# SUNGBEOMCHOI/Rubiks-Cube-Solver

Hardware: NVIDIA B200
Metric: cube transitions/sec (higher is better)
Workload: dtype u8

## Files before the change

rubiks_cube_solver_b200/csrc/cube_sched.cuh:

```cuda
#pragma once
#include <cstdint>
#include <cuda_runtime.h>

namespace sched {

constexpr int kClaimChunk = 2;
constexpr int kRanges = 8;
constexpr int kTailDiv = 4;
constexpr int kSlots = 1024;
constexpr int kExhausted = 0x7fffff00;

struct Slot { unsigned next[kRanges][32]; unsigned ctas_done; unsigned tail_div; unsigned pad[30]; };

Slot* claim_slot();
int tail_div();

struct WarpTiles {
    Slot* slot;
    int n_tiles, total_warps, tail0;
    int next_static;
    int r, visited;
    int cur, end;
    int chunk;
    unsigned pending;

    __device__ __forceinline__ int lo(int range) const
    {
        return tail0 + (int)((long long)range * (n_tiles - tail0) / kRanges);
    }
    __device__ __forceinline__ void claim_ahead(int lane)
    {
        if (lane == 0) pending = atomicAdd(&slot->next[r][0], (unsigned)chunk);
    }

    __device__ __forceinline__ void init(Slot* s, int n, int warps_per_cta, int warp, int lane, int tail_div,
                                         int claim_chunk = kClaimChunk)
    {
        slot = s; n_tiles = n; total_warps = (int)gridDim.x * warps_per_cta; chunk = claim_chunk;
        const int gid = (int)blockIdx.x * warps_per_cta + warp;
        tail0 = tail_div > 0 ? n - n / tail_div : n;
        next_static = gid;
        r = gid % kRanges; visited = 0; cur = end = 0; pending = 0;
        if (next_static >= tail0) claim_ahead(lane);
    }

    __device__ __forceinline__ int pop(int lane)
    {
        if (next_static < tail0) {
            const int t = next_static;
            next_static += total_warps;
            if (next_static >= tail0) claim_ahead(lane);
            return t;
        }
        while (cur >= end) {
            if (visited >= kRanges) return kExhausted;
            const unsigned got = __shfl_sync(0xffffffffu, pending, 0);
            const int hi = lo(r + 1);
            const long long base = (long long)lo(r) + got;
            if (base < hi) {
                cur = (int)base;
                end = cur + chunk < hi ? cur + chunk : hi;
            } else {
                bool left = false;
                if (lane < kRanges) left = lo(lane) + (long long)__ldcg(&slot->next[lane][0]) < lo(lane + 1);
                const unsigned open = __ballot_sync(0xffffffffu, left) & ((1u << kRanges) - 1u);
                if (open == 0) { visited = kRanges; return kExhausted; }
                const unsigned rot = (open >> (r + 1)) | (open << (kRanges - r - 1));
                r = (r + 1 + (__ffs(rot & ((1u << kRanges) - 1u)) - 1)) % kRanges;
            }
            claim_ahead(lane);
        }
        return cur++;
    }
};

__device__ __forceinline__ void release(Slot* slot)
{
    if (threadIdx.x == 0) {
        __threadfence();
        if (atomicAdd(&slot->ctas_done, 1u) == gridDim.x - 1) {
            for (int i = 0; i < kRanges; ++i) slot->next[i][0] = 0;
            slot->ctas_done = 0;
            __threadfence();
        }
    }
}

}
```

rubiks_cube_solver_b200/csrc/cube_threads.cuh:

```cuda
#pragma once
#include <cstdlib>
#include "cube_common.cuh"

template <int SIZE>
CUBE_HD void scramble_apply_word(CubieState& st, const uint32_t* s_tbl, uint32_t w)
{
    const uint32_t w4 = (w * 4u) & 0x3c3c3c3cu;
#pragma unroll
    for (int k = 0; k < 4; ++k) cubie_move_at<SIZE>(st, s_tbl, cube_prmt(w4, 0u, 0x4440u + k));
}

template <int SIZE>
CUBE_HD void scramble_run_staged(CubieState& st, int tid, int depth, const uint8_t* s_moves, const uint32_t* s_tbl)
{
    const uint32_t* mw = reinterpret_cast<const uint32_t*>(s_moves);
    const uint32_t r = (uint32_t)tid * (uint32_t)depth;
    const uint32_t wi = r >> 2, sh = (r & 3u) << 3;
    const int nfull = depth >> 2, tail = depth & 3;
    uint32_t lo = mw[wi];
#pragma unroll 2
    for (int j = 0; j < nfull; ++j) {
        const uint32_t hi = mw[wi + j + 1];
        const uint32_t w = cube_funnel_r(lo, hi, sh);
        lo = hi;
// ... 190 lines not shown
        const uint32_t m0 = cube_prmt(s.e0, t0, cube_hi16(Q.x)) ^ (P.w & 0x10101010u);
        const uint32_t m1 = cube_prmt(s.e1, t1, cube_hi16(Q.y)) ^ Q.w;
        const uint32_t m2 = cube_prmt(s.e2, t2, cube_hi16(Q.z)) ^ (P.w & 0x20202020u);
        s.e0 = m0; s.e1 = m1; s.e2 = m2;
    } else {
        uint32_t sel, t0w;
        tbl.ld64(addr, sel, t0w);
        const uint32_t t1w = tbl.ld32(addr + roff);
        const uint32_t n0 = cube_prmt(s.c0, s.c1, sel) + t0w;
        const uint32_t n1 = cube_prmt(s.c0, s.c1, cube_hi16(sel)) + t1w;
        s.c0 = n0; s.c1 = n1;
    }
}

template <int SIZE, int DEPTH>
CUBE_HD constexpr int pair_static_shift(int k)
{
    return DEPTH <= 0 ? -1
         : SIZE == 3 ? ((2 * DEPTH) % 4 == 0 ? ((k * DEPTH) % 4) * 8 : -1)
                     : (DEPTH % 4 == 0 ? 0 : -1);
}

template <int SSH>
CUBE_HD uint32_t pair_rows_word(uint32_t lo, uint32_t hi, uint32_t sh)
{
    constexpr uint32_t K = (uint32_t)(CUBE_PAIR_BASE + 256);
    if (SSH == 0) return lo * K;
    if (SSH == 16) return hi * (K << 16) + cube_hi16(lo) * K;
    return cube_funnel_r(lo, hi, sh) * K;
}

template <int SIZE, int DEPTH, int NS, class TBL>
CUBE_HD void scramble_pairs_run(CubieState (&st)[NS], const int (&rows)[NS], int depth_rt, const uint8_t* s_moves,
                                const TBL& tbl, uint32_t lanereg, uint32_t roff)
{
    const int depth = DEPTH > 0 ? DEPTH : depth_rt;
    const uint32_t* mw = reinterpret_cast<const uint32_t*>(s_moves);
    const int nfull = depth >> 2, tail = depth & 3;
    uint32_t wi[NS], sh[NS], lo[NS];
#pragma unroll
    for (int k = 0; k < NS; ++k) {
        const uint32_t r = (uint32_t)rows[k] * (uint32_t)depth;
        wi[k] = r >> 2; sh[k] = (r & 3u) << 3;
        lo[k] = mw[wi[k]];
    }
    auto word = [&](int j) {
        uint32_t y[NS];
        static_assert(NS == 1 || NS % 2 == 0, "instances come in pairs");
        if (SIZE == 3 || NS <= 2) {
            {
                constexpr int s0 = (NS >= 2) ? pair_static_shift<SIZE, DEPTH>(0) : -1;
#pragma unroll
                for (int h = 0; h < NS; h += 2) {
                    const uint32_t hi = (s0 == 0) ? 0u : mw[wi[h] + j + 1];
                    y[h] = pair_rows_word<s0>(lo[h], hi, sh[h]);
                    lo[h] = (s0 == 0) ? mw[wi[h] + j + 1] : hi;
                }
            }
            if (NS >= 2) {
                constexpr int s1 = pair_static_shift<SIZE, DEPTH>(1);
#pragma unroll
                for (int h = 1; h < NS; h += 2) {
                    const uint32_t hi = (s1 == 0) ? 0u : mw[wi[h] + j + 1];
                    y[h] = pair_rows_word<s1>(lo[h], hi, sh[h]);
                    lo[h] = (s1 == 0) ? mw[wi[h] + j + 1] : hi;
                }
            }
        } else {
            constexpr int s = pair_static_shift<2, DEPTH>(0);
#pragma unroll
            for (int k = 0; k < NS; ++k) {
                const uint32_t hi = (s == 0) ? 0u : mw[wi[k] + j + 1];
                y[k] = pair_rows_word<s>(lo[k], hi, sh[k]);
                lo[k] = (s == 0) ? mw[wi[k] + j + 1] : hi;
            }
        }
#pragma unroll
        for (int k = 0; k < NS; ++k) pair_apply<SIZE>(st[k], tbl, pair_addr<0>(y[k], lanereg), roff);
#pragma unroll
        for (int k = 0; k < NS; ++k) pair_apply<SIZE>(st[k], tbl, pair_addr<1>(y[k], lanereg), roff);
    };
    auto fold = [&]() {
#pragma unroll
        for (int k = 0; k < NS; ++k) {
            st[k].c0 = cubie_fold_twist(st[k].c0);
            st[k].c1 = cubie_fold_twist(st[k].c1);
        }
    };
    if (DEPTH > 0) {
#pragma unroll
        for (int j = 0; j < DEPTH / 4; ++j) {
            word(j);
            if (DEPTH > 30 && (j % 5 == 4 || j == DEPTH / 4 - 1)) fold();
        }
    } else {
        int j = 0;
        for (; j + 5 <= nfull; j += 5) {
            word(j); word(j + 1); word(j + 2); word(j + 3); word(j + 4);
            fold();
        }
        for (; j < nfull; ++j) word(j);
    }
    if (tail) {
        const uint32_t keep = (1u << (8 * tail)) - 1u;
        uint32_t y[NS];
#pragma unroll
        for (int k = 0; k < NS; ++k) {
            const uint32_t w = (cube_funnel_r(lo[k], mw[wi[k] + nfull + 1], sh[k]) & keep) | (0x0c0c0c0cu & ~keep);
            y[k] = w * (uint32_t)(CUBE_PAIR_BASE + 256);
        }
#pragma unroll
        for (int k = 0; k < NS; ++k) pair_apply<SIZE>(st[k], tbl, pair_addr<0>(y[k], lanereg), roff);
        if (tail == 3) {
#pragma unroll
            for (int k = 0; k < NS; ++k) pair_apply<SIZE>(st[k], tbl, pair_addr<1>(y[k], lanereg), roff);
        }
    }
}

template <int SIZE, int NS, class TBL>
CUBE_HD void scramble_pairs_run_units(CubieState (&st)[NS], const uint32_t (&base)[NS], const uint32_t (&shift)[NS], int len,
                                      const uint8_t* s_moves, const TBL& tbl, uint32_t lanereg, uint32_t roff)
{
    constexpr uint32_t K = (uint32_t)(CUBE_PAIR_BASE + 256);
    auto fold = [&]() {
#pragma unroll
        for (int k = 0; k < NS; ++k) {
            st[k].c0 = cubie_fold_twist(st[k].c0);
            st[k].c1 = cubie_fold_twist(st[k].c1);
        }
    };
    auto word = [&](const uint32_t (&w)[NS], bool second) {
        uint32_t y[NS];
#pragma unroll
        for (int k = 0; k < NS; ++k) y[k] = w[k] * K;
#pragma unroll
        for (int k = 0; k < NS; ++k) pair_apply<SIZE>(st[k], tbl, pair_addr<0>(y[k], lanereg), roff);
        if (second) {
#pragma unroll
            for (int k = 0; k < NS; ++k) pair_apply<SIZE>(st[k], tbl, pair_addr<1>(y[k], lanereg), roff);
        }
    };
    auto aligned = [&](const CubeVec4& a, const CubeVec4& b, uint32_t sh, uint32_t (&o)[4]) {
        const bool q0 = (sh & 4u) != 0, q1 = (sh & 8u) != 0;
        const uint32_t c[8] = {a.x, a.y, a.z, a.w, b.x, b.y, b.z, b.w};
        uint32_t e[7], d[5];
#pragma unroll
        for (int j = 0; j < 7; ++j) e[j] = q0 ? c[j + 1] : c[j];
#pragma unroll
        for (int j = 0; j < 5; ++j) d[j] = q1 ? e[j + 2] : e[j];
        const uint32_t r = (sh & 3u) << 3;
#pragma unroll
        for (int j = 0; j < 4; ++j) o[j] = cube_funnel_r(d[j], d[j + 1], r);
    };
    fold();
    CubeVec4 cur[NS];
#pragma unroll
    for (int k = 0; k < NS; ++k) cur[k] = cube_ld128(s_moves + base[k]);
    int g = 0;
    for (; g + 16 <= len; g += 16) {
        CubeVec4 nxt[NS];
        uint32_t m[NS][4], w[NS];
#pragma unroll
        for (int k = 0; k < NS; ++k) {
            nxt[k] = cube_ld128(s_moves + base[k] + g + 16);
            aligned(cur[k], nxt[k], shift[k], m[k]);
            cur[k] = nxt[k];
        }
#pragma unroll
        for (int j = 0; j < 4; ++j) {
#pragma unroll
            for (int k = 0; k < NS; ++k) w[k] = m[k][j];
            word(w, true);
        }
        fold();
    }
    const int rem = len - g;
    if (rem) {
        uint32_t m[NS][4], w[NS];
#pragma unroll
        for (int k = 0; k < NS; ++k) {
            const CubeVec4 nxt = cube_ld128(s_moves + base[k] + g + 16);
            aligned(cur[k], nxt, shift[k], m[k]);
        }
        const int nwords = rem >> 2, tail = rem & 3;
#pragma unroll
        for (int j = 0; j < 3; ++j) {
            if (j < nwords) {
#pragma unroll
                for (int k = 0; k < NS; ++k) w[k] = m[k][j];
                word(w, true);
            }
        }
        if (tail) {
            const uint32_t keep = (1u << (8 * tail)) - 1u;
#pragma unroll
            for (int k = 0; k < NS; ++k) {
                const uint32_t t = nwords == 0 ? m[k][0] : nwords == 1 ? m[k][1] : nwords == 2 ? m[k][2] : m[k][3];
                w[k] = (t & keep) | (0x0c0c0c0cu & ~keep);
            }
            word(w, tail == 3);
        }
    }
}

template <int SIZE, class TBL>
CUBE_HD void scramble_pairs_last(CubieState& st, uint32_t action, const TBL& tbl, uint32_t lanereg, uint32_t roff)
{
    st.c0 = cubie_fold_twist(st.c0);
    st.c1 = cubie_fold_twist(st.c1);
    const uint32_t y = (action | 0x0c0c0c00u) * (uint32_t)(CUBE_PAIR_BASE + 256);
    pair_apply<SIZE>(st, tbl, pair_addr<0>(y, lanereg), roff);
}

CUBE_HD uint32_t cube_swz128(uint32_t f) { return f ^ ((f >> 3) & 0x70u); }

template <int SIZE, int NS, class TBL>
CUBE_HD void scramble_pairs_run_swizzled(CubieState (&st)[NS], const uint8_t* tile, int lane, int depth, const TBL& tbl,
                                         uint32_t lanereg, uint32_t roff)
{
    constexpr uint32_t K = (uint32_t)(CUBE_PAIR_BASE + 256);
    static_assert(SIZE == 2 || NS == 2, "3x3x3: two rows per lane");
    auto word = [&](const uint32_t (&w)[NS]) {
        uint32_t y[NS];
#pragma unroll
        for (int k = 0; k < NS; ++k) y[k] = w[k] * K;
#pragma unroll
        for (int k = 0; k < NS; ++k) pair_apply<SIZE>(st[k], tbl, pair_addr<0>(y[k], lanereg), roff);
#pragma unroll
        for (int k = 0; k < NS; ++k) pair_apply<SIZE>(st[k], tbl, pair_addr<1>(y[k], lanereg), roff);
    };
    auto fold = [&]() {
#pragma unroll
        for (int k = 0; k < NS; ++k) {
            st[k].c0 = cubie_fold_twist(st[k].c0);
            st[k].c1 = cubie_fold_twist(st[k].c1);
        }
    };
    auto unit = [&](uint32_t f) { return cube_ld128(tile + cube_swz128(f)); };
    if (SIZE == 3 && (depth & 8)) {
        const int a = depth >> 4;
        const uint32_t f0 = (uint32_t)(lane * 2 * depth);
        CubeVec4 p = unit(f0 + 16 * a);
        const uint32_t last0[2] = {p.x, p.y};
        auto word2 = [&](uint32_t w0, uint32_t w1) {
            uint32_t w[NS];
            w[0] = w0; w[NS - 1] = w1;
            word(w);
        };
        for (int g = 0; g < a; ++g) {
            const CubeVec4 v = unit(f0 + 16 * g), q = unit(f0 + 16 * (a + g + 1));
            word2(v.x, p.z);
            word2(v.y, p.w);
            word2(v.z, q.x);
            word2(v.w, q.y);
            p = q;
            fold();
        }
        word2(last0[0], p.z);
        word2(last0[1], p.w);
        return;
    }
    uint32_t f[NS];
#pragma unroll
    for (int k = 0; k < NS; ++k) f[k] = (uint32_t)((SIZE == 3 ? 2 * lane + k : lane + 32 * k) * depth);
    for (int g = 0; g < depth; g += 16) {
        CubeVec4 v[NS];
#pragma unroll
        for (int k = 0; k < NS; ++k) v[k] = unit(f[k] + g);
        uint32_t w[NS];
#pragma unroll
        for (int k = 0; k < NS; ++k) w[k] = v[k].x;
        word(w);
#pragma unroll
        for (int k = 0; k < NS; ++k) w[k] = v[k].y;
        word(w);
#pragma unroll
        for (int k = 0; k < NS; ++k) w[k] = v[k].z;
        word(w);
#pragma unroll
        for (int k = 0; k < NS; ++k) w[k] = v[k].w;
        word(w);
        fold();
    }
}

CUBE_HD uint32_t cube_shr1(uint32_t x)
{
#if defined(__CUDA_ARCH__)
    uint32_t r;
    asm("mul.hi.u32 %0, %1, 2147483648;" : "=r"(r) : "r"(x));
    return r;
#else
    return x >> 1;
#endif
}

CUBE_HD uint32_t cubie_canonical_flip(uint32_t e)
{
    return ((cube_shr1(e) & 0x10101010u) ^ e) & 0x1f1f1f1fu;
}

template <int SIZE, class LUT>
CUBE_HD bool scramble_pairs_finish(CubieState& st, int row, const LUT& lut, uint8_t* s_out)
{
    st.c0 = cubie_reduce_twist(st.c0);
    st.c1 = cubie_reduce_twist(st.c1);
    bool ok = (st.c0 == 0x03020100u) & (st.c1 == 0x07060504u);
    uint32_t L[20];
#pragma unroll
    for (int q = 0; q < 4; ++q) {
        L[q] = lut.corner(st.c0, q);
        L[4 + q] = lut.corner(st.c1, q);
    }
    if (SIZE == 3) {
        const uint32_t f0 = cubie_canonical_flip(st.e0), f1 = cubie_canonical_flip(st.e1), f2 = cubie_canonical_flip(st.e2);
        ok = ok && ((f0 == 0x03020100u) & (f1 == 0x07060504u) & (f2 == 0x0b0a0908u));
        L[8] = lut.template edge<0>(f0);   L[9] = lut.template edge<1>(f0);   L[10] = lut.template edge<2>(f0);  L[11] = lut.template edge<3>(f0);
        L[12] = lut.template edge<4>(f1);  L[13] = lut.template edge<5>(f1);  L[14] = lut.template edge<6>(f1);  L[15] = lut.template edge<7>(f1);
        L[16] = lut.template edge<8>(f2);  L[17] = lut.template edge<9>(f2);  L[18] = lut.template edge<10>(f2); L[19] = lut.template edge<11>(f2);
        uint32_t w[13], h;
        uint8_t* rowp = s_out + 54 * row;
        if (row & 1) {
            cube_assemble3_odd(L, w, &h);
            *reinterpret_cast<uint16_t*>(rowp) = (uint16_t)h;
            uint32_t* wb = reinterpret_cast<uint32_t*>(rowp + 2);
#pragma unroll
            for (int j = 0; j < 13; ++j) wb[j] = w[j];
        } else {
            cube_assemble3_even(L, w, &h);
            uint32_t* wb = reinterpret_cast<uint32_t*>(rowp);
#pragma unroll
            for (int j = 0; j < 13; ++j) wb[j] = w[j];
            *reinterpret_cast<uint16_t*>(rowp + 52) = (uint16_t)h;
        }
    } else {
        uint32_t w[6];
        cube_assemble2(L, w);
        uint64_t* rowp = reinterpret_cast<uint64_t*>(s_out + 24 * row);
#pragma unroll
        for (int j = 0; j < 3; ++j) rowp[j] = (uint64_t)w[2 * j] | ((uint64_t)w[2 * j + 1] << 32);
    }
    return ok;
}

template <int SIZE>
CUBE_HD uint32_t pair_row_bit(uint32_t m0, uint32_t m1, int row)
{
    if (SIZE == 3) return (((row & 1) ? m1 : m0) >> (row >> 1)) & 1u;
    return (((row & 32) ? m1 : m0) >> (row & 31)) & 1u;
}

template <int SIZE>
CUBE_HD uint32_t pair_solved_word(uint32_t m0, uint32_t m1, int k)
{
    return pair_row_bit<SIZE>(m0, m1, 4 * k) | pair_row_bit<SIZE>(m0, m1, 4 * k + 1) << 8 |
           pair_row_bit<SIZE>(m0, m1, 4 * k + 2) << 16 | pair_row_bit<SIZE>(m0, m1, 4 * k + 3) << 24;
}

template <int SIZE>
CUBE_HD void walk_turn(uint8_t* row, uint32_t m, const uint32_t* s_cyc)
{
#pragma unroll
    for (int c = 0; c < CubeGeom<SIZE>::NCYC; ++c) {
        const uint32_t w = s_cyc[c * CUBE_MOVE_ROWS + m];
        const uint32_t a = w & 0xffu, b = (w >> 8) & 0xffu, cc = (w >> 16) & 0xffu, d = w >> 24;
        const uint8_t vb = row[b], vc = row[cc], vd = row[d], va = row[a];
        row[a] = vb; row[b] = vc; row[cc] = vd; row[d] = va;
    }
}

template <int SIZE>
CUBE_HD bool row_solved(const uint8_t* row)
{
    constexpr int S = CubeGeom<SIZE>::S, K = S / 6;
    const uint16_t* h = reinterpret_cast<const uint16_t*>(row);
    uint32_t diff = 0;
    uint32_t prev = 0;
#pragma unroll
    for (int i = 0; i < S / 2; ++i) {
        const uint32_t cur = h[i];
        const uint32_t b0 = cur & 0xffu, b1 = cur >> 8;
        if ((2 * i) % K != 0) diff |= b0 ^ prev;
        if ((2 * i + 1) % K != 0) diff |= b1 ^ b0;
        prev = b1;
    }
    return diff == 0;
}


template <int SIZE> struct WalkImage { static constexpr int W = (SIZE == 3) ? 14 : 6; };

CUBE_HD uint32_t walk_private_off(int k) { return (uint32_t)((k >> 2) * 128 + (k & 3)); }

CUBE_HD void walk_cycle_entry(uint32_t cw, int shift, uint32_t* e)
{
    const int a = (int)(cw & 0xffu) + shift, b = (int)((cw >> 8) & 0xffu) + shift;
    const int c = (int)((cw >> 16) & 0xffu) + shift, d = (int)(cw >> 24) + shift;
    e[0] = walk_private_off(a) | walk_private_off(b) << 16;
    e[1] = walk_private_off(c) | walk_private_off(d) << 16;
}

template <int SIZE>
CUBE_HD void walk_turn_private(uint8_t* lane_base, const uint32_t* ent, uint32_t m)
{
#pragma unroll
    for (int c = 0; c < CubeGeom<SIZE>::NCYC; ++c) {
        const uint32_t w0 = ent[(c * CUBE_MOVE_ROWS + m) * 2], w1 = ent[(c * CUBE_MOVE_ROWS + m) * 2 + 1];
        const uint32_t a = w0 & 0xffffu, b = cube_hi16(w0), cc = w1 & 0xffffu, d = cube_hi16(w1);
        const uint8_t vb = lane_base[b], vc = lane_base[cc], vd = lane_base[d], va = lane_base[a];
        lane_base[a] = vb; lane_base[b] = vc; lane_base[cc] = vd; lane_base[d] = va;
    }
}

template <int A>
CUBE_HD void walk_select_child2(const uint32_t* p, uint32_t m, uint32_t* out)
{
    uint32_t c[6];
    cube_child2<A>(p, c);
#pragma unroll
    for (int j = 0; j < 6; ++j) out[j] = (m == (uint32_t)A) ? c[j] : out[j];
}

CUBE_HD void walk_turn_registers2(uint32_t* w, uint32_t m)
{
    uint32_t out[6];
#pragma unroll
    for (int j = 0; j < 6; ++j) out[j] = w[j];
    walk_select_child2<0>(w, m, out);
    walk_select_child2<1>(w, m, out);
    walk_select_child2<2>(w, m, out);
    walk_select_child2<3>(w, m, out);
    walk_select_child2<4>(w, m, out);
    walk_select_child2<5>(w, m, out);
#pragma unroll
    for (int j = 0; j < 6; ++j) w[j] = out[j];
}

template <int SIZE, int SHIFT>
CUBE_HD bool image_solved(const uint32_t* w)
{
    constexpr int S = CubeGeom<SIZE>::S, K = S / 6, W = WalkImage<SIZE>::W;
    uint32_t acc = 0;
#pragma unroll
    for (int j = 0; j < W; ++j) {
        uint32_t mask = 0;
#pragma unroll
        for (int k = 0; k < 4; ++k) {
            const int i = 4 * j + k - SHIFT;
            if (i >= 1 && i < S && (i % K) != 0) mask |= 0xffu << (8 * k);
        }
        if (mask) {
            const uint32_t prev = (j == 0) ? (w[0] << 8) : ((w[j] << 8) | (w[j - 1] >> 24));
            acc |= (w[j] ^ prev) & mask;
        }
    }
    return acc == 0;
}

template <int DTYPE> struct OneHot;
template <> struct OneHot<0> { static constexpr int V = 8, ESIZE = 2; };
template <> struct OneHot<1> { static constexpr int V = 4, ESIZE = 4; };
template <> struct OneHot<2> { static constexpr int V = 16, ESIZE = 1; };

template <int DTYPE>
CUBE_HD void onehot_set(uint32_t* w, int p)
{
    if (DTYPE == 0) {
        const uint32_t v = (p & 1) ? 0x3f800000u : 0x00003f80u;
#pragma unroll
        for (int q = 0; q < 4; ++q) w[q] |= ((p >> 1) == q) ? v : 0u;
    } else if (DTYPE == 1) {
#pragma unroll
        for (int q = 0; q < 4; ++q) w[q] |= (p == q) ? 0x3f800000u : 0u;
    } else {
        const uint32_t v = 1u << (8 * (p & 3));
#pragma unroll
        for (int q = 0; q < 4; ++q) w[q] |= ((p >> 2) == q) ? v : 0u;
    }
}

template <int DTYPE, int C>
CUBE_HD void onehot_vector_at(int seg, int off, const uint8_t* col, uint32_t* w)
{
    w[0] = w[1] = w[2] = w[3] = 0u;
    onehot_set<DTYPE>(w, (int)col[seg] - off);
    if (C % OneHot<DTYPE>::V != 0) onehot_set<DTYPE>(w, C - off + (int)col[seg + 1]);
}

template <int DTYPE, int C>
CUBE_HD void onehot_vector(int v, const uint8_t* col, int n_seg, uint32_t* w)
{
    (void)n_seg;
    const int e0 = v * OneHot<DTYPE>::V;
    const int seg = e0 / C;
    onehot_vector_at<DTYPE, C>(seg, e0 - seg * C, col, w);
}

template <int SIZE>
CUBE_HD uint32_t onehot_code(const uint8_t* row, int slot, const uint32_t* s_def, const uint8_t* s_lut0,
                             const uint8_t* s_lut1)
{
    const uint32_t d = s_def[slot];
    const uint32_t a = row[d & 0xffu], b = row[(d >> 8) & 0xffu], c = row[(d >> 16) & 0xffu];
    if (SIZE == 3 && slot >= 8) return s_lut1[(a + 10u * b) & 127u];
    return s_lut0[(a + 2u * b + 10u * c) & 127u];
}
```

rubiks_cube_solver_b200/csrc/scramble.cu:

```cuda
#include <cstring>
#include <cuda.h>
#include <cuda_runtime.h>
#include "cube_bulk.cuh"
#include "cube_kernels.h"
#include "cube_launch.cuh"
#include "cube_sched.cuh"
#include "cube_threads.cuh"

namespace {

#ifndef CUBE_SCRAMBLE_MIN_BLOCKS
#define CUBE_SCRAMBLE_MIN_BLOCKS 6
#endif
constexpr int kTile = 256;
constexpr int kMaxStagedDepth = 160;

__host__ __device__ constexpr int round16(int x) { return (x + 15) & ~15; }

template <int SIZE>
struct ScrambleSmem {
    using G = CubeGeom<SIZE>;
    static constexpr int kTable = 0;
    static constexpr int kCornerLut = kTable + G::MW * CUBE_MOVE_ROWS * 4;
    static constexpr int kEdgeLut = kCornerLut + 32 * 4;
    static constexpr int kBarrier = kEdgeLut + 64 * 4;
    static constexpr int kFlags = kBarrier + 16;
    static constexpr int kOut = round16(kFlags + kTile);
    static constexpr int kMoves = kOut + round16(kTile * G::S);
    __host__ __device__ static constexpr int bytes(int depth, bool staged)
    {
        return kMoves + (staged ? round16(kTile * depth) + 32 : 0);
    }
};

template <int SIZE>
__device__ __forceinline__ void load_tables(uint8_t* smem, int tid)
{
    using L = ScrambleSmem<SIZE>;
    uint32_t* s_tbl = reinterpret_cast<uint32_t*>(smem + L::kTable);
    uint32_t* s_clut = reinterpret_cast<uint32_t*>(smem + L::kCornerLut);
    uint32_t* s_elut = reinterpret_cast<uint32_t*>(smem + L::kEdgeLut);
    if (tid < CubeGeom<SIZE>::MW * CUBE_MOVE_ROWS) s_tbl[tid] = (SIZE == 3) ? kMoveWords3[tid] : kMoveWords2[tid];
    if (tid >= 128 && tid < 160) s_clut[tid - 128] = (SIZE == 3) ? kCornerColour3[tid - 128] : kCornerColour2[tid - 128];
    if (tid >= 160 && tid < 224) s_elut[tid - 160] = (SIZE == 3) ? kEdgeColour3[tid - 160] : 0u;
}

template <int SIZE, bool FULL>
__global__ void __launch_bounds__(kTile, CUBE_SCRAMBLE_MIN_BLOCKS)
scramble_tile_kernel(const uint8_t* __restrict__ moves, long long n, long long tile0, int depth,
                     uint8_t* __restrict__ out, uint8_t* __restrict__ solved, float* __restrict__ reward,
                     unsigned long long* __restrict__ counters, const uint8_t* __restrict__ last)
{
    using G = CubeGeom<SIZE>;
    using L = ScrambleSmem<SIZE>;
    extern __shared__ __align__(128) uint8_t smem[];
    const uint32_t* s_tbl = reinterpret_cast<const uint32_t*>(smem + L::kTable);
    const uint32_t* s_clut = reinterpret_cast<const uint32_t*>(smem + L::kCornerLut);
    const uint32_t* s_elut = reinterpret_cast<const uint32_t*>(smem + L::kEdgeLut);
    uint64_t* s_bar = reinterpret_cast<uint64_t*>(smem + L::kBarrier);
    uint8_t* s_flags = smem + L::kFlags;
    uint8_t* s_out = smem + L::kOut;
    uint8_t* s_moves = smem + L::kMoves;

    const int tid = threadIdx.x;
    const int row = (SIZE == 3) ? 2 * (((tid >> 5) & 3) * 32 + (tid & 31)) + (tid >> 7) : tid;
    const long long base = (tile0 + blockIdx.x) * kTile;
    const int cnt = FULL ? kTile : (int)(n - base);
    constexpr bool full = FULL;
    const uint32_t move_bytes = (uint32_t)(kTile * depth);

    if (full && depth > 0 && tid == 0) {
        bulk::mbar_init(s_bar, 1);
        bulk::mbar_expect_tx(s_bar, move_bytes);
        bulk::load(s_moves, moves + base * depth, move_bytes, s_bar);
    }
    load_tables<SIZE>(smem, tid);
    if (!full) {
        const long long byte0 = base * depth;
        const int nbytes = cnt * depth;
        for (int i = tid; i < nbytes; i += kTile) s_moves[i] = moves[byte0 + i];
    }
    __syncthreads();
    if (full && depth > 0) bulk::mbar_wait(s_bar, 0);

    bool ok = false;
    if (row < cnt) {
        CubieState st;
        cubie_init(st);
        scramble_run_staged<SIZE>(st, row, depth, s_moves, s_tbl);
        if (last) {
            st.c0 = cubie_fold_twist(st.c0); st.c1 = cubie_fold_twist(st.c1);
            cubie_move<SIZE>(st, s_tbl, (uint32_t)__ldg(last + base + row) & 0xfu);
        }
        ok = scramble_finish<SIZE>(st, row, s_clut, s_elut, s_out);
        s_flags[row] = ok ? 1 : 0;
    }
    const unsigned bal = __ballot_sync(0xffffffffu, ok);
    if ((tid & 31) == 0 && bal && counters) atomicAdd(&counters[0], (unsigned long long)__popc(bal));
    if (blockIdx.x == 0 && tid == 0 && counters) atomicAdd(&counters[1], (unsigned long long)(FULL ? (long long)gridDim.x * kTile : (long long)cnt));

    if (full) bulk::fence_smem_writes();
    __syncthreads();
    if (full) {
        if (tid == 0) {
            bulk::store(out + base * G::S, s_out, (uint32_t)(kTile * G::S));
            bulk::commit();
        }
    } else {
        const long long byte0 = base * G::S;
        const int nbytes = cnt * G::S;
        for (int i = tid; i < nbytes; i += kTile) out[byte0 + i] = s_out[i];
    }
    if (tid < cnt) {
        const bool row_ok = s_flags[tid] != 0;
        if (solved) solved[base + tid] = row_ok ? 1 : 0;
        if (reward) reward[base + tid] = row_ok ? 1.0f : -1.0f;
    }
    if (full && tid == 0) bulk::wait_read_all();
}


constexpr int kMaxPairDepth = 320;
constexpr int kPairTableBytes = CUBE_PAIR_ROWS * 256;
template <int SIZE, int NS> struct PairCfg;
template <> struct PairCfg<3, 2> { static constexpr int kMaxWarps = 24; };
template <> struct PairCfg<2, 2> { static constexpr int kMaxWarps = 32; };
template <> struct PairCfg<2, 4> { static constexpr int kMaxWarps = 20; };
constexpr int kMinWarpsFour = 16;

template <int SIZE, int NS>
struct PairSmem {
    using G = CubeGeom<SIZE>;
    static constexpr int kPairTile = 32 * NS;
    static constexpr int kTable = 0;
    static constexpr int kCornerLut = kPairTableBytes + 256;
    static constexpr int kEdgeLut = kCornerLut + 256;
    static constexpr int kPerWarp = (kEdgeLut + (SIZE == 3 ? 1536 : 256) + 1023) / 1024 * 1024;
    static constexpr int kOutBytes = kPairTile * G::S;
    __host__ __device__ static constexpr int round1k(int x) { return (x + 1023) & ~1023; }
    __host__ __device__ static constexpr int move_stride(int depth, bool swz = false)
    {
        return swz ? round1k(kPairTile * depth) : kPairTile * depth + 16;
    }
    __host__ __device__ static constexpr int moves_at(bool swz = false) { return swz ? round1k(16 + kOutBytes) : 16 + kOutBytes; }
    __host__ __device__ static constexpr int per_warp(int depth, bool swz = false)
    {
        return moves_at(swz) + 2 * move_stride(depth, swz);
    }
    __host__ __device__ static constexpr int bytes(int depth, int warps, bool priv = false)
    {
        return kPerWarp + warps * per_warp(depth, priv) < 66048 ? 66048 : kPerWarp + warps * per_warp(depth, priv);
    }
};

template <int SIZE, int DEPTH, int NS, int MODE>
__global__ void __launch_bounds__(PairCfg<SIZE, NS>::kMaxWarps * 32, 1)
scramble_pairs_kernel(const uint8_t* __restrict__ moves, int n_tiles, int depth_rt, uint8_t* __restrict__ out,
                      uint8_t* __restrict__ solved, float* __restrict__ reward, unsigned long long* __restrict__ counters,
                      sched::Slot* slot, int tail_div, const __grid_constant__ CUtensorMap move_map,
                      const uint8_t* __restrict__ last)
{
    using L = PairSmem<SIZE, NS>;
    constexpr int kPairTile = L::kPairTile;
    extern __shared__ __align__(128) uint8_t smem_raw[];
    const int depth = DEPTH > 0 ? DEPTH : depth_rt;
    constexpr bool kPriv = DEPTH < 0;
    constexpr uint32_t kAlign = kPriv ? 1024u : 256u;
    const int tid = threadIdx.x, lane = tid & 31, warp = tid >> 5;
    const uint32_t window = bulk::smem_addr(smem_raw);
    uint8_t* smem = smem_raw + ((kAlign - (window & (kAlign - 1u))) & (kAlign - 1u));
    uint8_t* s_ptbl = smem + L::kTable;
    const PairTableShared tbl{bulk::smem_addr(s_ptbl)};
    uint32_t* s_clut = reinterpret_cast<uint32_t*>(smem + L::kCornerLut);
    uint32_t* s_elut = reinterpret_cast<uint32_t*>(smem + L::kEdgeLut);
    uint8_t* mine = smem + L::kPerWarp + warp * L::per_warp(depth, kPriv);
    uint64_t* s_bar = reinterpret_cast<uint64_t*>(mine);
    uint8_t* s_out = mine + 16;
    uint8_t* s_moves = mine + L::moves_at(kPriv);
    const int mstride = L::move_stride(depth, kPriv);
    const uint32_t move_bytes = (uint32_t)(kPairTile * depth);
    auto stage = [&](int t, int b) {
        if (bulk::elect_one()) {
            bulk::mbar_expect_tx(&s_bar[b], move_bytes);
            if (!kPriv) bulk::load(s_moves + b * mstride, moves + (long long)t * move_bytes, move_bytes, &s_bar[b]);
            else bulk::load_tile_2d(s_moves + b * mstride, &move_map, 0, t * (kPairTile * depth >> 7), &s_bar[b]);
        }
    };

    asm volatile("griddepcontrol.launch_dependents;");
    pair_table_fill<SIZE>(s_ptbl, tid, blockDim.x);
    if (tid < 32) s_clut[tid] = (SIZE == 3) ? kCornerColour3[tid] : kCornerColour2[tid];
    if (SIZE == 3) for (int i = tid; i < 12 * 32; i += blockDim.x) s_elut[i] = kEdgeColourSlot3[i];
    if (lane == 0) { bulk::mbar_init(&s_bar[0], 1); bulk::mbar_init(&s_bar[1], 1); }
    if (lane == 0 && depth > 0) {
        const int total = (int)gridDim.x * (int)(blockDim.x >> 5);
#pragma unroll
        for (int k = 0; k < 2; ++k) {
            const int t = (int)blockIdx.x * (int)(blockDim.x >> 5) + warp + k * total;
            if (t < n_tiles) bulk::prefetch_l2(moves + (long long)t * move_bytes, move_bytes);
        }
    }
    __syncthreads();
    asm volatile("griddepcontrol.wait;" ::: "memory");

    sched::WarpTiles tiles;
    tiles.init(slot, n_tiles, (int)(blockDim.x >> 5), warp, lane, tail_div);
    int tile = tiles.pop(lane);
    if (tile < n_tiles) stage(tile, 0);
    int rows[NS];
#pragma unroll
    for (int k = 0; k < NS; ++k) rows[k] = (SIZE == 3) ? 64 * (k >> 1) + 2 * lane + (k & 1) : lane + 32 * k;
    const uint32_t lanereg = pair_lanereg<SIZE>(lane, tbl), roff = pair_roff2(lane);
    const ColourLutShared lut{bulk::smem_addr(s_clut), bulk::smem_addr(s_elut)};
    unsigned n_solved = 0;
    const bool has_last = MODE == 2 || (MODE == 0 && last != nullptr);
    const bool has_solved = MODE != 0 || solved != nullptr, has_reward = MODE != 0 || reward != nullptr;
    for (int it = 0; tile < n_tiles; ++it) {
        const int buf = it & 1;
        const int next = tiles.pop(lane);
        if (next < n_tiles) stage(next, buf ^ 1);
        uint32_t last_w[NS];
        if (has_last) {
            if (SIZE == 3) {
#pragma unroll
                for (int h = 0; h < NS; h += 2) {
                    const uint32_t v = *reinterpret_cast<const uint16_t*>(last + (long long)tile * kPairTile + 32 * h + 2 * lane);
                    last_w[h] = v & 0xffu; last_w[h + 1] = v >> 8;
                }
            } else {
#pragma unroll
                for (int k = 0; k < NS; ++k) last_w[k] = last[(long long)tile * kPairTile + 32 * k + lane];
            }
        }
        bulk::mbar_wait(&s_bar[buf], (uint32_t)(it >> 1) & 1u);

        CubieState st[NS];
#pragma unroll
        for (int k = 0; k < NS; ++k) cubie_init(st[k]);
        if constexpr (kPriv) scramble_pairs_run_swizzled<SIZE, NS>(st, s_moves + buf * mstride, lane, depth, tbl, lanereg, roff);
        else scramble_pairs_run<SIZE, (DEPTH > 0 ? DEPTH : 0), NS>(st, rows, depth, s_moves + buf * mstride, tbl, lanereg, roff);
        if (has_last) {
#pragma unroll
            for (int k = 0; k < NS; ++k) scramble_pairs_last<SIZE>(st[k], last_w[k], tbl, lanereg, roff);
        }
        if (bulk::elect_one()) bulk::wait_read_all();
        __syncwarp();
        bool ok[NS];
#pragma unroll
        for (int k = 0; k < NS; ++k) {
            ok[k] = scramble_pairs_finish<SIZE>(st[k], rows[k], lut, s_out);
            n_solved += ok[k] ? 1u : 0u;
        }

        bulk::fence_smem_writes();
        __syncwarp();
        if (bulk::elect_one()) {
            bulk::store(out + (long long)tile * L::kOutBytes, s_out, (uint32_t)L::kOutBytes);
            bulk::commit();
        }
        if (SIZE == 3) {
#pragma unroll
            for (int h = 0; h < NS; h += 2) {
                const long long r0 = (long long)tile * kPairTile + 32 * h + 2 * lane;
                if (has_solved) *reinterpret_cast<uint16_t*>(solved + r0) = (uint16_t)((ok[h] ? 1u : 0u) | (ok[h + 1] ? 0x100u : 0u));
                if (has_reward) *reinterpret_cast<float2*>(reward + r0) = make_float2(ok[h] ? 1.0f : -1.0f, ok[h + 1] ? 1.0f : -1.0f);
            }
        } else {
#pragma unroll
            for (int k = 0; k < NS; ++k) {
                if (has_solved) solved[(long long)tile * kPairTile + 32 * k + lane] = ok[k] ? 1 : 0;
                if (has_reward) reward[(long long)tile * kPairTile + 32 * k + lane] = ok[k] ? 1.0f : -1.0f;
            }
        }
        tile = next;
    }
    n_solved = __reduce_add_sync(0xffffffffu, n_solved);
    if (lane == 0 && n_solved && counters) atomicAdd(&counters[0], (unsigned long long)n_solved);
    if (blockIdx.x == 0 && tid == 0 && counters) atomicAdd(&counters[1], (unsigned long long)n_tiles * kPairTile);
    __syncwarp();
    if (bulk::elect_one()) bulk::wait_read_all();
    __syncthreads();
    sched::release(slot);
}

constexpr int kSliceDefault = 112;
__host__ __device__ constexpr int slice_stride(int slice) { return ((slice + 32) / 16) % 2 ? slice + 32 : slice + 48; }

template <int SIZE>
struct SlicedSmem {
    using G = CubeGeom<SIZE>;
    static constexpr int kOutBytes = 64 * G::S;
    static constexpr int kMovesAt = 16 + kOutBytes;
    __host__ __device__ static constexpr int per_warp(int slice) { return kMovesAt + 2 * 64 * slice_stride(slice); }
    static constexpr int kFixed = PairSmem<SIZE, 2>::kPerWarp;
    __host__ __device__ static constexpr int bytes(int warps, int slice) { return kFixed + warps * per_warp(slice); }
};

template <int SIZE>
__global__ void __launch_bounds__(8 * 32, 1)
scramble_sliced_kernel(const uint8_t* __restrict__ moves, int n_tiles, int depth, uint8_t* __restrict__ out,
                       uint8_t* __restrict__ solved, float* __restrict__ reward, unsigned long long* __restrict__ counters,
                       const uint8_t* __restrict__ last, int kSlice)
{
    using L = SlicedSmem<SIZE>;
    using P = PairSmem<SIZE, 2>;
    extern __shared__ __align__(128) uint8_t smem_raw[];
    const int tid = threadIdx.x, lane = tid & 31, warp = tid >> 5, warps = (int)(blockDim.x >> 5);
    const uint32_t window = bulk::smem_addr(smem_raw);
    uint8_t* smem = smem_raw + ((256u - (window & 255u)) & 255u);
    uint8_t* s_ptbl = smem + P::kTable;
    const PairTableShared tbl{bulk::smem_addr(s_ptbl)};
    uint32_t* s_clut = reinterpret_cast<uint32_t*>(smem + P::kCornerLut);
    uint32_t* s_elut = reinterpret_cast<uint32_t*>(smem + P::kEdgeLut);
    const int kSliceStride = slice_stride(kSlice);
    uint8_t* mine = smem + L::kFixed + warp * L::per_warp(kSlice);
    uint64_t* s_bar = reinterpret_cast<uint64_t*>(mine);
    uint8_t* s_out = mine + 16;
    uint8_t* s_moves = mine + L::kMovesAt;

    pair_table_fill<SIZE>(s_ptbl, tid, blockDim.x);
    if (tid < 32) s_clut[tid] = (SIZE == 3) ? kCornerColour3[tid] : kCornerColour2[tid];
    if (SIZE == 3) for (int i = tid; i < 12 * 32; i += blockDim.x) s_elut[i] = kEdgeColourSlot3[i];
    if (lane == 0) { bulk::mbar_init(&s_bar[0], 32); bulk::mbar_init(&s_bar[1], 32); }
    __syncthreads();

    const int n_slices = (depth + kSlice - 1) / kSlice;
    const int rows[2] = {lane, lane + 32};
    const uint32_t shift[2] = {(uint32_t)(((long long)rows[0] * depth) & 15), (uint32_t)(((long long)rows[1] * depth) & 15)};
    auto stage = [&](int t, int s, int b) {
        const int len = depth - s * kSlice < kSlice ? depth - s * kSlice : kSlice;
        uint32_t bytes[2];
#pragma unroll
        for (int k = 0; k < 2; ++k) bytes[k] = (shift[k] + (uint32_t)len + 15u) & ~15u;
        bulk::mbar_expect_tx(&s_bar[b], bytes[0] + bytes[1]);
#pragma unroll
        for (int k = 0; k < 2; ++k) {
            const long long g = ((long long)t * 64 + rows[k]) * depth + (long long)s * kSlice;
            bulk::load(s_moves + (b * 64 + rows[k]) * kSliceStride, moves + (g & ~15LL), bytes[k], &s_bar[b]);
        }
    };
    const uint32_t lanereg = pair_lanereg<SIZE>(lane, tbl), roff = pair_roff2(lane);
    const ColourLutShared lut{bulk::smem_addr(s_clut), bulk::smem_addr(s_elut)};
    unsigned n_solved = 0;
    const int stride = (int)gridDim.x * warps;
    int tile = (int)blockIdx.x * warps + warp;
    if (tile < n_tiles) stage(tile, 0, 0);
    for (unsigned it = 0; tile < n_tiles; tile += stride) {
        CubieState st[2];
        cubie_init(st[0]);
        cubie_init(st[1]);
        for (int s = 0; s < n_slices; ++s, ++it) {
            const int buf = (int)(it & 1u);
            __syncwarp();
            if (s + 1 < n_slices) stage(tile, s + 1, buf ^ 1);
            else if (tile + stride < n_tiles) stage(tile + stride, 0, buf ^ 1);
            bulk::mbar_wait(&s_bar[buf], (it >> 1) & 1u);
            const int len = depth - s * kSlice < kSlice ? depth - s * kSlice : kSlice;
            const uint32_t base[2] = {(uint32_t)((buf * 64 + rows[0]) * kSliceStride), (uint32_t)((buf * 64 + rows[1]) * kSliceStride)};
            scramble_pairs_run_units<SIZE, 2>(st, base, shift, len, s_moves, tbl, lanereg, roff);
        }
        if (last) {
#pragma unroll
            for (int k = 0; k < 2; ++k)
                scramble_pairs_last<SIZE>(st[k], (uint32_t)__ldg(last + (long long)tile * 64 + rows[k]), tbl, lanereg, roff);
        }
        if (lane == 0) bulk::wait_read_all();
        __syncwarp();
        bool ok[2];
#pragma unroll
        for (int k = 0; k < 2; ++k) {
            ok[k] = scramble_pairs_finish<SIZE>(st[k], rows[k], lut, s_out);
            n_solved += ok[k] ? 1u : 0u;
        }
        bulk::fence_smem_writes();
        __syncwarp();
        if (lane == 0) {
            bulk::store(out + (long long)tile * L::kOutBytes, s_out, (uint32_t)L::kOutBytes);
            bulk::commit();
        }
#pragma unroll
        for (int k = 0; k < 2; ++k) {
            if (solved) solved[(long long)tile * 64 + rows[k]] = ok[k] ? 1 : 0;
            if (reward) reward[(long long)tile * 64 + rows[k]] = ok[k] ? 1.0f : -1.0f;
        }
    }
    n_solved = __reduce_add_sync(0xffffffffu, n_solved);
    if (lane == 0 && n_solved && counters) atomicAdd(&counters[0], (unsigned long long)n_solved);
    if (blockIdx.x == 0 && tid == 0 && counters) atomicAdd(&counters[1], (unsigned long long)n_tiles * 64);
    if (lane == 0) bulk::wait_read_all();
}

template <int SIZE>
long long launch_sliced(const uint8_t* moves, long long n, int depth, uint8_t* out, uint8_t* solved, float* reward,
                        unsigned long long* counters, cudaStream_t stream, const uint8_t* last)
{
    using L = SlicedSmem<SIZE>;
    long long n_tiles = n / 64 - 1;
    if (n_tiles < 1) return 0;
    if (n_tiles > 0x3fffffff) n_tiles = 0x3fffffff;
    static const int slice = [] {
        const int v = cube::env_int("CUBE_SLICE", kSliceDefault);
        return (v >= 16 && v <= 240 && v % 16 == 0) ? v : kSliceDefault;
    }();
    int warps = cube::warps_that_fit(256 + L::kFixed, L::per_warp(slice), 8);
    if (warps >= 4) warps &= ~3;
    if (warps < 1) return 0;
    const int smem = L::bytes(warps, slice) + 256 < 66048 + 256 ? 66048 + 256 : L::bytes(warps, slice) + 256;
    auto kern = scramble_sliced_kernel<SIZE>;
    cudaError_t e = cube::raise_smem_limit(kern, smem);
    if (e != cudaSuccess) return -(long long)e;
    kern<<<cube::persistent_grid(n_tiles, warps), warps * 32, smem, stream>>>(moves, (int)n_tiles, depth, out, solved, reward,
                                                                            counters, last, slice);
    e = cudaGetLastError();
    if (e != cudaSuccess) return -(long long)e;
    return n_tiles * 64;
}

template <int SIZE>
__global__ void __launch_bounds__(kTile, 4)
scramble_deep_kernel(const uint8_t* __restrict__ moves, long long n, int depth, uint8_t* __restrict__ out,
                     uint8_t* __restrict__ solved, float* __restrict__ reward,
                     unsigned long long* __restrict__ counters, const uint8_t* __restrict__ last)
{
    using G = CubeGeom<SIZE>;
    using L = ScrambleSmem<SIZE>;
    extern __shared__ __align__(128) uint8_t smem[];
    const uint32_t* s_tbl = reinterpret_cast<const uint32_t*>(smem + L::kTable);
    const uint32_t* s_clut = reinterpret_cast<const uint32_t*>(smem + L::kCornerLut);
    const uint32_t* s_elut = reinterpret_cast<const uint32_t*>(smem + L::kEdgeLut);
    uint8_t* s_out = smem + L::kOut;
    const int tid = threadIdx.x;
    load_tables<SIZE>(smem, tid);

    const long long n_tiles = (n + kTile - 1) / kTile;
    for (long long tile = blockIdx.x; tile < n_tiles; tile += gridDim.x) {
        const long long base = tile * kTile;
        const int cnt = (int)((n - base) < (long long)kTile ? (n - base) : (long long)kTile);
        __syncthreads();
        bool ok = false;
        if (tid < cnt) {
            CubieState st;
            cubie_init(st);
            const uint8_t* row = moves + (base + tid) * depth;
            for (int k = 0; k < depth; ++k) {
                cubie_move<SIZE>(st, s_tbl, (uint32_t)__ldg(row + k) & 0xfu);
                if ((k & 3) == 3) { st.c0 = cubie_fold_twist(st.c0); st.c1 = cubie_fold_twist(st.c1); }
            }
            if (last) {
                st.c0 = cubie_fold_twist(st.c0); st.c1 = cubie_fold_twist(st.c1);
                cubie_move<SIZE>(st, s_tbl, (uint32_t)__ldg(last + base + tid) & 0xfu);
            }
            ok = scramble_finish<SIZE>(st, tid, s_clut, s_elut, s_out);
            if (solved) solved[base + tid] = ok ? 1 : 0;
            if (reward) reward[base + tid] = ok ? 1.0f : -1.0f;
        }
        const unsigned bal = __ballot_sync(0xffffffffu, ok);
        if ((tid & 31) == 0 && bal && counters) atomicAdd(&counters[0], (unsigned long long)__popc(bal));
        __syncthreads();
        const long long byte0 = base * G::S;
        const int nbytes = cnt * G::S;
        const int nvec = nbytes >> 4;
        int4* dst = reinterpret_cast<int4*>(out + byte0);
        for (int i = tid; i < nvec; i += kTile) __stcs(dst + i, reinterpret_cast<const int4*>(s_out)[i]);
        for (int i = (nvec << 4) + tid; i < nbytes; i += kTile) out[byte0 + i] = s_out[i];
    }
    if (blockIdx.x == 0 && tid == 0 && counters) atomicAdd(&counters[1], (unsigned long long)n);
}

template <int SIZE>
int launch_classic(const uint8_t* moves, long long n, int depth, uint8_t* out, uint8_t* solved, float* reward,
                   unsigned long long* counters, cudaStream_t stream, const uint8_t* last)
{
    const bool staged = depth <= kMaxStagedDepth;
    const int smem = ScrambleSmem<SIZE>::bytes(depth, staged);
    const long long n_tiles = (n + kTile - 1) / kTile;
    if (staged) {
        auto kern_full = scramble_tile_kernel<SIZE, true>;
        auto kern_tail = scramble_tile_kernel<SIZE, false>;
        cudaError_t e = cube::raise_smem_limit(kern_full, smem);
        if (e == cudaSuccess) e = cube::raise_smem_limit(kern_tail, smem);
        if (e != cudaSuccess) return (int)e;
        cube::prefer_max_shared(kern_full);
        const long long full_tiles = n / kTile;
        if (full_tiles > 0)
            kern_full<<<(unsigned)full_tiles, kTile, smem, stream>>>(moves, n, 0, depth, out, solved, reward, counters, last);
        if (full_tiles < n_tiles)
            kern_tail<<<1, kTile, smem, stream>>>(moves, n, full_tiles, depth, out, solved, reward, counters, last);
    } else {
        auto kern = scramble_deep_kernel<SIZE>;
        int per_sm = 0;
        if (cudaOccupancyMaxActiveBlocksPerMultiprocessor(&per_sm, kern, kTile, smem) != cudaSuccess || per_sm < 1)
            per_sm = 1;
        long long grid = (long long)cube::sm_count() * per_sm;
        if (grid > n_tiles) grid = n_tiles;
        kern<<<(unsigned)grid, kTile, smem, stream>>>(moves, n, depth, out, solved, reward, counters, last);
    }
    return (int)cudaGetLastError();
}

using EncodeTiledFn = CUresult (*)(CUtensorMap*, CUtensorMapDataType, cuuint32_t, void*, const cuuint64_t*,
                                   const cuuint64_t*, const cuuint32_t*, const cuuint32_t*, CUtensorMapInterleave,
                                   CUtensorMapSwizzle, CUtensorMapL2promotion, CUtensorMapFloatOOBfill);

bool encode_move_map(CUtensorMap* map, const uint8_t* moves, long long n_tiles, int tile_rows)
{
    static const EncodeTiledFn encode = [] {
        void* p = nullptr;
        cudaDriverEntryPointQueryResult q = cudaDriverEntryPointSymbolNotFound;
        if (cudaGetDriverEntryPoint("cuTensorMapEncodeTiled", &p, cudaEnableDefault, &q) != cudaSuccess ||
            q != cudaDriverEntryPointSuccess)
            p = nullptr;
        (void)cudaGetLastError();
        return reinterpret_cast<EncodeTiledFn>(p);
    }();
    if (!encode) return false;
    const cuuint64_t dims[2] = {128, (cuuint64_t)(n_tiles * tile_rows)};
    const cuuint64_t strides[1] = {128};
    const cuuint32_t box[2] = {128, (cuuint32_t)tile_rows};
    const cuuint32_t elem[2] = {1, 1};
    return encode(map, CU_TENSOR_MAP_DATA_TYPE_UINT8, 2, const_cast<uint8_t*>(moves), dims, strides, box, elem,
                  CU_TENSOR_MAP_INTERLEAVE_NONE, CU_TENSOR_MAP_SWIZZLE_128B, CU_TENSOR_MAP_L2_PROMOTION_NONE,
                  CU_TENSOR_MAP_FLOAT_OOB_FILL_NONE) == CUDA_SUCCESS;
}

template <int SIZE, int NS>
long long launch_pairs(const uint8_t* moves, long long n, int depth, uint8_t* out, uint8_t* solved, float* reward,
                       unsigned long long* counters, cudaStream_t stream, int min_warps, const uint8_t* last)
{
    using L = PairSmem<SIZE, NS>;
    constexpr int kPairTile = L::kPairTile;
    if (n < kPairTile) return 0;
    static const bool swz_ok = cube::env_flag("CUBE_PAIR_SWIZZLE", true);
    static_assert(L::kPerWarp % 1024 == 0, "the per-warp areas of the swizzled variant start on 1 KB");
    long long n_tiles = n / kPairTile;
    if (n_tiles > 0x3fffffff) n_tiles = 0x3fffffff;
    const int tile_rows = kPairTile * depth / 128;
    constexpr bool kCanSwizzle = SIZE == 2 || NS == 2;
    bool priv = kCanSwizzle && swz_ok && depth % (SIZE == 3 ? 8 : 16) == 0 && n_tiles * tile_rows < 0x7fffffffLL;
    auto warps_for = [&](bool p) {
        return cube::warps_that_fit((p ? 1024 : 256) + L::kPerWarp, L::per_warp(depth, p), PairCfg<SIZE, NS>::kMaxWarps) & ~3;
    };
    if (warps_for(priv) < min_warps) return 0;
    alignas(64) CUtensorMap move_map;
    memset(&move_map, 0, sizeof(move_map));
    if (priv && !encode_move_map(&move_map, moves, n_tiles, tile_rows)) priv = false;
    const int slack = priv ? 1024 : 256;
    const int warps = warps_for(priv);
    if (warps < min_warps) return 0;
    const int smem = L::bytes(depth, warps, priv) + slack;
    constexpr int kM2 = SIZE == 3 ? 2 : 0;
    const int mode = (solved && reward) ? (last ? kM2 : 1) : 0;
    const int variant = depth == 30 ? 1 : depth == 20 ? 2 : priv ? 3 : 0;
    using Kern = decltype(&scramble_pairs_kernel<SIZE, 0, NS, 0>);
    constexpr int kSwz = kCanSwizzle ? -1 : 0;
    static const Kern kerns[3][4] = {
        {scramble_pairs_kernel<SIZE, 0, NS, 0>, scramble_pairs_kernel<SIZE, 30, NS, 0>, scramble_pairs_kernel<SIZE, 20, NS, 0>, scramble_pairs_kernel<SIZE, kSwz, NS, 0>},
        {scramble_pairs_kernel<SIZE, 0, NS, 1>, scramble_pairs_kernel<SIZE, 30, NS, 1>, scramble_pairs_kernel<SIZE, 20, NS, 1>, scramble_pairs_kernel<SIZE, kSwz, NS, 1>},
        {scramble_pairs_kernel<SIZE, 0, NS, kM2>, scramble_pairs_kernel<SIZE, 30, NS, kM2>, scramble_pairs_kernel<SIZE, 20, NS, kM2>, scramble_pairs_kernel<SIZE, kSwz, NS, kM2>}};
    const Kern kern = kerns[mode][variant];
    cudaError_t e = cube::raise_smem_limit(kern, smem);
    if (e != cudaSuccess) return -(long long)e;
    sched::Slot* slot = sched::claim_slot();
    if (!slot) return -(long long)cudaErrorUnknown;
    e = cube::launch_pdl(kern, cube::persistent_grid(n_tiles, warps), warps * 32, smem, stream, moves, (int)n_tiles, depth,
                         out, solved, reward, counters, slot, sched::tail_div(), move_map, last);
    if (e != cudaSuccess) return -(long long)e;
    return n_tiles * kPairTile;
}

template <int SIZE>
int launch_one(const uint8_t* moves, long long n, int depth, uint8_t* out, uint8_t* solved, float* reward,
               unsigned long long* counters, cudaStream_t stream, const uint8_t* last)
{
    using G = CubeGeom<SIZE>;
    long long done = 0;
    static const bool classic = cube::env_flag("CUBE_SCRAMBLE_CLASSIC", false);
    static const bool four_ok = cube::env_flag("CUBE_PAIR_FOUR", true);
// ... 32 lines not shown
```

Baseline: 1426 billion.

## Split tail tiles into half-tiles in the dynamic scheduler for finer load balance

The work-stealing scheduler now represents the last tiles of each range as two half-tile units, so warps near the end of the grid can claim half a pair-tile (32 rows) instead of a whole one. The kernel gains a half-tile path that stages half the move bytes, runs one cube per lane, and writes its colour rows through a new runtime-parity assembly routine. The aim is to shrink tail imbalance across warps. The cost is extra scheduler arithmetic, smaller claims near the tail, and a less efficient single-state path for those units.

```diff
diff --git a/rubiks_cube_solver_b200/csrc/cube_sched.cuh b/rubiks_cube_solver_b200/csrc/cube_sched.cuh
--- a/rubiks_cube_solver_b200/csrc/cube_sched.cuh
+++ b/rubiks_cube_solver_b200/csrc/cube_sched.cuh
@@ -7,6 +7,10 @@
 constexpr int kClaimChunk = 2;
 constexpr int kRanges = 8;
 constexpr int kTailDiv = 4;
+#ifndef CUBE_SPLIT_TILES_PER_WARP
+#define CUBE_SPLIT_TILES_PER_WARP 2
+#endif
+constexpr int kSplitTilesPerWarp = CUBE_SPLIT_TILES_PER_WARP;
 constexpr int kSlots = 1024;
 constexpr int kExhausted = 0x7fffff00;
 
@@ -22,55 +26,79 @@
     int r, visited;
     int cur, end;
     int chunk;
+    int split;
+    int claim;
     unsigned pending;
 
     __device__ __forceinline__ int lo(int range) const
     {
         return tail0 + (int)((long long)range * (n_tiles - tail0) / kRanges);
     }
-    __device__ __forceinline__ void claim_ahead(int lane)
+    __device__ __forceinline__ int whole(int range) const
     {
-        if (lane == 0) pending = atomicAdd(&slot->next[r][0], (unsigned)chunk);
+        const int w = lo(range + 1) - lo(range);
+        return w > split ? w - split : 0;
+    }
+    __device__ __forceinline__ int units(int range) const
+    {
+        const int w = lo(range + 1) - lo(range);
+        return 2 * w - (w > split ? w - split : 0);
+    }
+    __device__ __forceinline__ void claim_ahead(int lane, int n)
+    {
+        claim = n;
+        if (lane == 0) pending = atomicAdd(&slot->next[r][0], (unsigned)n);
     }
 
     __device__ __forceinline__ void init(Slot* s, int n, int warps_per_cta, int warp, int lane, int tail_div,
-                                         int claim_chunk = kClaimChunk)
+                                         bool halves = false, int claim_chunk = kClaimChunk)
     {
         slot = s; n_tiles = n; total_warps = (int)gridDim.x * warps_per_cta; chunk = claim_chunk;
+        split = halves ? (kSplitTilesPerWarp * total_warps + kRanges - 1) / kRanges : 0;
         const int gid = (int)blockIdx.x * warps_per_cta + warp;
         tail0 = tail_div > 0 ? n - n / tail_div : n;
         next_static = gid;
         r = gid % kRanges; visited = 0; cur = end = 0; pending = 0;
-        if (next_static >= tail0) claim_ahead(lane);
+        if (next_static >= tail0) claim_ahead(lane, chunk);
     }
 
-    __device__ __forceinline__ int pop(int lane)
+    __device__ __forceinline__ int pop(int lane, int& part)
     {
+        part = 0;
         if (next_static < tail0) {
             const int t = next_static;
             next_static += total_warps;
-            if (next_static >= tail0) claim_ahead(lane);
+            if (next_static >= tail0) claim_ahead(lane, chunk);
             return t;
         }
         while (cur >= end) {
             if (visited >= kRanges) return kExhausted;
             const unsigned got = __shfl_sync(0xffffffffu, pending, 0);
-            const int hi = lo(r + 1);
-            const long long base = (long long)lo(r) + got;
-            if (base < hi) {
-                cur = (int)base;
-                end = cur + chunk < hi ? cur + chunk : hi;
+            const int u = units(r);
+            bool in_range = false;
+            if (got < (unsigned)u) {
+                cur = (int)got;
+                end = cur + claim < u ? cur + claim : u;
+                in_range = true;
             } else {
                 bool left = false;
-                if (lane < kRanges) left = lo(lane) + (long long)__ldcg(&slot->next[lane][0]) < lo(lane + 1);
+                if (lane < kRanges) left = __ldcg(&slot->next[lane][0]) < (unsigned)units(lane);
                 const unsigned open = __ballot_sync(0xffffffffu, left) & ((1u << kRanges) - 1u);
                 if (open == 0) { visited = kRanges; return kExhausted; }
                 const unsigned rot = (open >> (r + 1)) | (open << (kRanges - r - 1));
                 r = (r + 1 + (__ffs(rot & ((1u << kRanges) - 1u)) - 1)) % kRanges;
             }
-            claim_ahead(lane);
+            claim_ahead(lane, in_range && end + chunk <= whole(r) ? chunk : 1);
         }
-        return cur++;
+        const int u = cur++, w = whole(r);
+        if (u < w) return lo(r) + u;
+        part = 1 + ((u - w) & 1);
+        return lo(r) + w + ((u - w) >> 1);
+    }
+    __device__ __forceinline__ int pop(int lane)
+    {
+        int part;
+        return pop(lane, part);
     }
 };
 
diff --git a/rubiks_cube_solver_b200/csrc/cube_threads.cuh b/rubiks_cube_solver_b200/csrc/cube_threads.cuh
--- a/rubiks_cube_solver_b200/csrc/cube_threads.cuh
+++ b/rubiks_cube_solver_b200/csrc/cube_threads.cuh
@@ -516,12 +516,11 @@
 }
 
 template <int SIZE, class LUT>
-CUBE_HD bool scramble_pairs_finish(CubieState& st, int row, const LUT& lut, uint8_t* s_out)
+CUBE_HD bool pair_finish_lookup(CubieState& st, const LUT& lut, uint32_t (&L)[20])
 {
     st.c0 = cubie_reduce_twist(st.c0);
     st.c1 = cubie_reduce_twist(st.c1);
     bool ok = (st.c0 == 0x03020100u) & (st.c1 == 0x07060504u);
-    uint32_t L[20];
 #pragma unroll
     for (int q = 0; q < 4; ++q) {
         L[q] = lut.corner(st.c0, q);
@@ -533,6 +532,16 @@
         L[8] = lut.template edge<0>(f0);   L[9] = lut.template edge<1>(f0);   L[10] = lut.template edge<2>(f0);  L[11] = lut.template edge<3>(f0);
         L[12] = lut.template edge<4>(f1);  L[13] = lut.template edge<5>(f1);  L[14] = lut.template edge<6>(f1);  L[15] = lut.template edge<7>(f1);
         L[16] = lut.template edge<8>(f2);  L[17] = lut.template edge<9>(f2);  L[18] = lut.template edge<10>(f2); L[19] = lut.template edge<11>(f2);
+    }
+    return ok;
+}
+
+template <int SIZE, class LUT>
+CUBE_HD bool scramble_pairs_finish(CubieState& st, int row, const LUT& lut, uint8_t* s_out)
+{
+    uint32_t L[20];
+    const bool ok = pair_finish_lookup<SIZE>(st, lut, L);
+    if (SIZE == 3) {
         uint32_t w[13], h;
         uint8_t* rowp = s_out + 54 * row;
         if (row & 1) {
@@ -555,6 +564,22 @@
 #pragma unroll
         for (int j = 0; j < 3; ++j) rowp[j] = (uint64_t)w[2 * j] | ((uint64_t)w[2 * j + 1] << 32);
     }
+    return ok;
+}
+
+template <class LUT>
+CUBE_HD bool scramble_pairs_finish_rt(CubieState& st, int row, const LUT& lut, uint8_t* s_out)
+{
+    uint32_t L[20];
+    const bool ok = pair_finish_lookup<3>(st, lut, L);
+    uint32_t w[14];
+    cube_assemble3_even(L, w, &w[13]);
+    const uint32_t odd = (uint32_t)row & 1u, sh = odd << 4;
+    uint8_t* rowp = s_out + 54 * row;
+    uint32_t* wb = reinterpret_cast<uint32_t*>(rowp + 2 * odd);
+#pragma unroll
+    for (int j = 0; j < 13; ++j) wb[j] = cube_funnel_r(w[j], w[j + 1], sh);
+    *reinterpret_cast<uint16_t*>(rowp + (odd ? 0 : 52)) = (uint16_t)(odd ? w[0] : w[13]);
     return ok;
 }
 
diff --git a/rubiks_cube_solver_b200/csrc/scramble.cu b/rubiks_cube_solver_b200/csrc/scramble.cu
--- a/rubiks_cube_solver_b200/csrc/scramble.cu
+++ b/rubiks_cube_solver_b200/csrc/scramble.cu
@@ -11,6 +11,9 @@
 
 #ifndef CUBE_SCRAMBLE_MIN_BLOCKS
 #define CUBE_SCRAMBLE_MIN_BLOCKS 6
+#endif
+#ifndef CUBE_K1P_CHUNK
+#define CUBE_K1P_CHUNK 2
 #endif
 constexpr int kTile = 256;
 constexpr int kMaxStagedDepth = 160;
@@ -179,10 +182,12 @@
     uint8_t* s_moves = mine + L::moves_at(kPriv);
     const int mstride = L::move_stride(depth, kPriv);
     const uint32_t move_bytes = (uint32_t)(kPairTile * depth);
-    auto stage = [&](int t, int b) {
+    constexpr bool kHalves = SIZE == 3 && NS == 2 && !kPriv;
+    auto stage = [&](int t, int p, int b) {
         if (bulk::elect_one()) {
-            bulk::mbar_expect_tx(&s_bar[b], move_bytes);
-            if (!kPriv) bulk::load(s_moves + b * mstride, moves + (long long)t * move_bytes, move_bytes, &s_bar[b]);
+            const uint32_t bytes = kHalves && p ? move_bytes >> 1 : move_bytes;
+            bulk::mbar_expect_tx(&s_bar[b], bytes);
+            if (!kPriv) bulk::load(s_moves + b * mstride, moves + (long long)t * move_bytes + (p == 2 ? bytes : 0u), bytes, &s_bar[b]);
             else bulk::load_tile_2d(s_moves + b * mstride, &move_map, 0, t * (kPairTile * depth >> 7), &s_bar[b]);
         }
     };
@@ -204,9 +209,10 @@
     asm volatile("griddepcontrol.wait;" ::: "memory");
 
     sched::WarpTiles tiles;
-    tiles.init(slot, n_tiles, (int)(blockDim.x >> 5), warp, lane, tail_div);
-    int tile = tiles.pop(lane);
-    if (tile < n_tiles) stage(tile, 0);
+    tiles.init(slot, n_tiles, (int)(blockDim.x >> 5), warp, lane, tail_div, kHalves, CUBE_K1P_CHUNK);
+    int part = 0;
+    int tile = tiles.pop(lane, part);
+    if (tile < n_tiles) stage(tile, part, 0);
     int rows[NS];
 #pragma unroll
     for (int k = 0; k < NS; ++k) rows[k] = (SIZE == 3) ? 64 * (k >> 1) + 2 * lane + (k & 1) : lane + 32 * k;
@@ -215,10 +221,38 @@
     unsigned n_solved = 0;
     const bool has_last = MODE == 2 || (MODE == 0 && last != nullptr);
     const bool has_solved = MODE != 0 || solved != nullptr, has_reward = MODE != 0 || reward != nullptr;
+    auto half_tile = [&](int t, int p, int b, int i) {
+        const long long r0 = (long long)t * kPairTile + 32 * (p - 1);
+        const uint32_t last_h = has_last ? (uint32_t)last[r0 + lane] : 0u;
+        bulk::mbar_wait(&s_bar[b], (uint32_t)(i >> 1) & 1u);
+        CubieState sh[1];
+        cubie_init(sh[0]);
+        const int row[1] = {lane};
+        scramble_pairs_run<SIZE, (DEPTH > 0 ? DEPTH : 0), 1>(sh, row, depth, s_moves + b * mstride, tbl, lanereg, roff);
+        if (has_last) scramble_pairs_last<SIZE>(sh[0], last_h, tbl, lanereg, roff);
+        if (bulk::elect_one()) bulk::wait_read_all();
+        __syncwarp();
+        const bool ok = scramble_pairs_finish_rt(sh[0], lane, lut, s_out);
+        n_solved += ok ? 1u : 0u;
+        bulk::fence_smem_writes();
+        __syncwarp();
+        if (bulk::elect_one()) {
+            bulk::store(out + r0 * CubeGeom<SIZE>::S, s_out, (uint32_t)(L::kOutBytes / 2));
+            bulk::commit();
+        }
+        if (has_solved) solved[r0 + lane] = ok ? 1 : 0;
+        if (has_reward) reward[r0 + lane] = ok ? 1.0f : -1.0f;
+    };
     for (int it = 0; tile < n_tiles; ++it) {
         const int buf = it & 1;
-        const int next = tiles.pop(lane);
-        if (next < n_tiles) stage(next, buf ^ 1);
+        int next_part;
+        const int next = tiles.pop(lane, next_part);
+        if (next < n_tiles) stage(next, next_part, buf ^ 1);
+        if (kHalves && part) {
+            half_tile(tile, part, buf, it);
+            tile = next; part = next_part;
+            continue;
+        }
         uint32_t last_w[NS];
         if (has_last) {
             if (SIZE == 3) {
@@ -272,7 +306,7 @@
                 if (has_reward) reward[(long long)tile * kPairTile + 32 * k + lane] = ok[k] ? 1.0f : -1.0f;
             }
         }
-        tile = next;
+        tile = next; part = next_part;
     }
     n_solved = __reduce_add_sync(0xffffffffu, n_solved);
     if (lane == 0 && n_solved && counters) atomicAdd(&counters[0], (unsigned long long)n_solved);
```

Measured after the change: 1378 billion (median of 6 runs). 0.967x the previous value.
